# qingpowuwu/emd

Measured on AMD Instinct MI355X. Metric: train iters/s (fwd+bwd) @1066x1600, 2M Gaussians; 1/2/4/8 GPU, higher is better.
Workload: dtype f32

## Files before the change

### emd_amd/csrc/api.hip

```cpp
#include <stdarg.h>
#include <stdio.h>
#include <stdlib.h>
#include <string.h>

#include "common.h"

static thread_local char g_err[512] = "";

void emd_set_error(const char* fmt, ...) {
    va_list ap;
    va_start(ap, fmt);
    vsnprintf(g_err, sizeof(g_err), fmt, ap);
    va_end(ap);
}

#include <mutex>
#include <vector>
namespace {
struct ProfRec { int stage; hipEvent_t a, b; bool b_shared; };
bool g_prof_on = false;
std::mutex g_prof_mu;
std::vector<ProfRec> g_prof_recs;
std::vector<hipEvent_t> g_prof_pool;
hipEvent_t g_prof_open[EMD_PROF_STAGES];
// ... 145 lines not shown
const char* emd_last_error(void) { return g_err; }

int emd_raster_workspace_size(const EmdDims* dims, size_t out[4]) {
    if (!dims || !out) { emd_set_error("workspace_size: null argument"); return EMD_ERR_INVALID; }
    if (dims->num_gaussians < 0 || dims->image_height <= 0 || dims->image_width <= 0 || dims->bin_capacity < 0) {
        emd_set_error("workspace_size: bad dims N=%d H=%d W=%d cap=%lld", dims->num_gaussians, dims->image_height,
                      dims->image_width, (long long)dims->bin_capacity);
        return EMD_ERR_INVALID;
    }
    GeomWs g; BinWs b; ImgWs im;
    const int gx = (dims->image_width + EMD_TILE_X - 1) / EMD_TILE_X, gy = (dims->image_height + EMD_TILE_Y - 1) / EMD_TILE_Y;
    emd_carve_geom(nullptr, dims->num_gaussians, &g);
    emd_carve_bin(nullptr, dims->bin_capacity, gx * gy, &b);
    emd_carve_img(nullptr, dims->image_height, dims->image_width, &im);
    out[0] = g.bytes; out[1] = b.bytes; out[2] = im.bytes;
    if (dims->num_extra < 0 || dims->num_extra > EMD_MAX_EXTRA) { emd_set_error("workspace_size: num_extra %d not in 0..%d", dims->num_extra, EMD_MAX_EXTRA); return EMD_ERR_INVALID; }
    out[3] = (size_t)(dims->num_gaussians > 0 ? dims->num_gaussians : 1) * emd_bwd_stride(dims->num_extra) * sizeof(float);
    return EMD_OK;
}

static int check_common(const EmdSettings& s, int N, int M, const float* means3D, const float* shs,
                        const float* colors, const float* opac, const float* scales, const float* rots,
                        const float* cov, int flags, const EmdMotion& mo) {
    if (N < 0 || s.image_height <= 0 || s.image_width <= 0) { emd_set_error("bad sizes N=%d H=%d W=%d", N, s.image_height, s.image_width); return EMD_ERR_INVALID; }
    if (N > 0 && (!means3D || !opac)) { emd_set_error("means3D / opacities must not be null"); return EMD_ERR_INVALID; }
    if ((shs != nullptr) == (colors != nullptr) && N > 0) { emd_set_error("provide exactly one of shs / colors_precomp"); return EMD_ERR_INVALID; }
    const bool sr = scales && rots;
    if (((scales != nullptr) != (rots != nullptr)) || (sr == (cov != nullptr) && N > 0)) {
        emd_set_error("provide exactly one of (scales, rotations) / cov3D_precomp"); return EMD_ERR_INVALID;
    }
    if (s.sh_degree < 0 || s.sh_degree > 3) { emd_set_error("sh_degree %d not in 0..3", s.sh_degree); return EMD_ERR_INVALID; }
    if (shs && M < (s.sh_degree + 1) * (s.sh_degree + 1)) { emd_set_error("shs holds %d coefficients, degree %d needs %d", M, s.sh_degree, (s.sh_degree + 1) * (s.sh_degree + 1)); return EMD_ERR_INVALID; }
    if (!(flags & EMD_FLAG_SDEV_TANFOV) && (!(s.tanfovx > 0.f) || !(s.tanfovy > 0.f))) { emd_set_error("tanfov must be positive"); return EMD_ERR_INVALID; }
    if (flags & EMD_FLAG_MOTION) {
        if (mo.actor_id && (!mo.actor_pose || mo.num_actors <= 0)) { emd_set_error("motion: actor_id given without actor_pose"); return EMD_ERR_INVALID; }
        if (cov) { emd_set_error("motion: cov3D_precomp cannot be combined with the fused motion transform"); return EMD_ERR_INVALID; }
    }
    if ((flags & EMD_FLAG_RAW_PARAMS) && cov) { emd_set_error("raw params: cov3D_precomp has no raw form"); return EMD_ERR_INVALID; }
    return EMD_OK;
}

int emd_raster_forward(EmdFwdArgs* a, void* hip_stream) {
    if (!a) { emd_set_error("forward: null args"); return EMD_ERR_INVALID; }
    hipStream_t st = (hipStream_t)hip_stream;
    const int N = a->num_gaussians;
    int rc = check_common(a->s, N, a->sh_coeffs, a->means3D, a->shs, a->colors_precomp, a->opacities, a->scales,
                          a->rotations, a->cov3D_precomp, a->flags, a->motion);
    if (rc) return rc;
    if (!a->out_color || !a->out_depth || !a->out_alpha || !a->radii || !a->status || !a->geom_ws || !a->bin_ws || !a->img_ws) {
        emd_set_error("forward: null output / workspace pointer"); return EMD_ERR_INVALID;
    }
    if ((a->flags & EMD_FLAG_NORMAL) && !a->out_normal) { emd_set_error("forward: EMD_FLAG_NORMAL without out_normal"); return EMD_ERR_INVALID; }
    if (a->bin_capacity < 0) { emd_set_error("forward: negative bin_capacity"); return EMD_ERR_INVALID; }
    if ((int64_t)N >= (int64_t)1 << 28) { emd_set_error("forward: %d Gaussians; a list word holds a 28-bit Gaussian id beside the pair's quadrant mask", N); return EMD_ERR_INVALID; }
    if (a->num_extra < 0 || a->num_extra > EMD_MAX_EXTRA) { emd_set_error("forward: num_extra %d not in 0..%d", a->num_extra, EMD_MAX_EXTRA); return EMD_ERR_INVALID; }
    for (int k = 0; k < a->num_extra; k++)
        if (!a->colors_extra[k] || !a->out_extra[k]) { emd_set_error("forward: extra colour set %d: null colours / output", k); return EMD_ERR_INVALID; }
    if ((a->flags & EMD_FLAG_SDEV_TANFOV) && !a->settings_dev) { emd_set_error("forward: EMD_FLAG_SDEV_TANFOV without settings_dev"); return EMD_ERR_INVALID; }
    const int gx = (a->s.image_width + EMD_TILE_X - 1) / EMD_TILE_X, gy = (a->s.image_height + EMD_TILE_Y - 1) / EMD_TILE_Y;
    GeomWs g; BinWs b; ImgWs im;
    emd_carve_geom(a->geom_ws, N, &g);
    emd_carve_bin(a->bin_ws, a->bin_capacity, gx * gy, &b);
    emd_carve_img(a->img_ws, a->s.image_height, a->s.image_width, &im);
    if (g.bytes > a->geom_bytes || b.bytes > a->bin_bytes || im.bytes > a->img_bytes) {
        emd_set_error("forward: workspace too small (geom %zu/%zu bin %zu/%zu img %zu/%zu)", a->geom_bytes, g.bytes,
                      a->bin_bytes, b.bytes, a->img_bytes, im.bytes);
        return EMD_ERR_WORKSPACE;
    }
    const bool dbg = a->s.debug != 0;
#define STAGE_SYNC(name)                                                                                     \
    if (dbg) {                                                                                               \
        hipError_t e_ = hipStreamSynchronize(st);                                                            \
        if (e_ != hipSuccess) { emd_set_error("stage %s failed: %s", name, hipGetErrorString(e_)); return EMD_ERR_HIP; } \
    }
    PreArgs pa;
    pa.s = a->s; pa.N = N; pa.M = a->sh_coeffs; pa.flags = a->flags;
    pa.means3D = a->means3D; pa.shs = a->shs; pa.colors_precomp = a->colors_precomp; pa.opacities = a->opacities;
    pa.scales = a->scales; pa.rotations = a->rotations; pa.cov3D_precomp = a->cov3D_precomp;
    pa.motion = a->motion; pa.radii = a->radii; pa.g = g; pa.status = a->status; pa.sdev = a->settings_dev;
    pa.shs_res0 = a->shs_residual[0]; pa.shs_res1 = a->shs_residual[1];
    if ((pa.shs_res0 || pa.shs_res1) && !a->shs) { emd_set_error("raster_forward: shs_residual needs shs"); return EMD_ERR_INVALID; }
    if (pa.shs_res1 && !pa.shs_res0) { pa.shs_res0 = pa.shs_res1; pa.shs_res1 = nullptr; }
    if (!(a->flags & EMD_FLAG_MOTION)) memset(&pa.motion, 0, sizeof(pa.motion));
    emd_prof_begin(PROF_PREPROCESS, st);
    hipStream_t aux = (hipStream_t)a->aux_stream;
    const bool split = aux != nullptr && aux != st && N > 0 && !dbg;
    hipEvent_t ev_fork = nullptr, ev_join = nullptr;
    auto join = [&]() -> int {
        if (!ev_join) return EMD_OK;
        hipError_t e1 = hipStreamWaitEvent(st, ev_join, 0);
        (void)hipEventDestroy(ev_fork); (void)hipEventDestroy(ev_join);
        ev_fork = ev_join = nullptr;
        if (e1 != hipSuccess) { emd_set_error("forward: joining the auxiliary stream failed: %s", hipGetErrorString(e1)); return EMD_ERR_HIP; }
        return EMD_OK;
    };
    rc = emd_launch_preprocess(pa, split ? 1 : 0, st);
    if (rc) return rc;
    if (split) {
        EMD_HIP_CHECK(hipEventCreateWithFlags(&ev_fork, hipEventDisableTiming));
        EMD_HIP_CHECK(hipEventCreateWithFlags(&ev_join, hipEventDisableTiming));
        EMD_HIP_CHECK(hipEventRecord(ev_fork, st));
        EMD_HIP_CHECK(hipStreamWaitEvent(aux, ev_fork, 0));
        rc = emd_launch_preprocess(pa, 2, aux);
        hipError_t e2 = hipEventRecord(ev_join, aux);
        if (rc || e2 != hipSuccess) { (void)join(); if (!rc) { emd_set_error("forward: hipEventRecord on the auxiliary stream failed"); rc = EMD_ERR_HIP; } return rc; }
    }
    STAGE_SYNC("preprocess");
// ... 306 lines not shown
```

### emd_amd/csrc/footprint.h

```cpp
#pragma once
#include <hip/hip_runtime.h>

struct EllipseCull {
    float mx, my, A, C, kx, ky, nbc, nba, thr;
    bool none, all;
};
__device__ __forceinline__ EllipseCull ellipse_prepare(const float4& r0, const float4& r1) {
    EllipseCull e;
    const float o = r0.w;
    e.mx = r0.x; e.my = r0.y; e.A = r1.x; e.C = r1.z;
    e.none = !(o >= (1.f / 255.f));
    const float ac = r1.x * r1.z, det = ac - r1.y * r1.y;
    e.all = !(det > 0.f) || !(r1.x > 0.f) || !(r1.z > 0.f) || !(det * 3.0e4f > ac);
    e.thr = 2.f * __logf(255.f * o) * 1.01f + 0.05f;
    const float ia = __builtin_amdgcn_rcpf(r1.x), ic = __builtin_amdgcn_rcpf(r1.z);
    e.kx = det * ic; e.ky = det * ia; e.nbc = -r1.y * ic; e.nba = -r1.y * ia;
    return e;
}
__device__ __forceinline__ bool ellipse_hits_rect(const EllipseCull& e, float x0, float x1, float y0, float y1) {
    const float dxa = e.mx - x0, dxb = e.mx - x1, dya = e.my - y0, dyb = e.my - y1;
    const bool inside = dxa >= 0.f && dxb <= 0.f && dya >= 0.f && dyb <= 0.f;
    float ta = e.nbc * dxa, tb = e.nbc * dxb;
    float ea = __builtin_amdgcn_fmed3f(ta, dyb, dya) - ta, eb = __builtin_amdgcn_fmed3f(tb, dyb, dya) - tb;
    const float qa = __builtin_fmaf(e.C * ea, ea, (e.kx * dxa) * dxa), qb = __builtin_fmaf(e.C * eb, eb, (e.kx * dxb) * dxb);
    ta = e.nba * dya; tb = e.nba * dyb;
    ea = __builtin_amdgcn_fmed3f(ta, dxb, dxa) - ta; eb = __builtin_amdgcn_fmed3f(tb, dxb, dxa) - tb;
    const float qc = __builtin_fmaf(e.A * ea, ea, (e.ky * dya) * dya), qd = __builtin_fmaf(e.A * eb, eb, (e.ky * dyb) * dyb);
    const float q = fminf(fminf(qa, qb), fminf(qc, qd));
    return !e.none && (e.all || inside || q <= e.thr);
}
__device__ __forceinline__ uint32_t ellipse_subblock_mask(const float4& r0, const float4& r1, float qx0, float qy0) {
    const EllipseCull e = ellipse_prepare(r0, r1);
    return (ellipse_hits_rect(e, qx0, qx0 + 3.f, qy0, qy0 + 3.f) ? 1u : 0u) | (ellipse_hits_rect(e, qx0 + 4.f, qx0 + 7.f, qy0, qy0 + 3.f) ? 2u : 0u) |
           (ellipse_hits_rect(e, qx0, qx0 + 3.f, qy0 + 4.f, qy0 + 7.f) ? 4u : 0u) |
           (ellipse_hits_rect(e, qx0 + 4.f, qx0 + 7.f, qy0 + 4.f, qy0 + 7.f) ? 8u : 0u);
}
__device__ __forceinline__ uint32_t ellipse_quadrant_mask(const EllipseCull& e, float tx0, float ty0) {
    return (ellipse_hits_rect(e, tx0, tx0 + 7.f, ty0, ty0 + 7.f) ? 1u : 0u) | (ellipse_hits_rect(e, tx0 + 8.f, tx0 + 15.f, ty0, ty0 + 7.f) ? 2u : 0u) |
           (ellipse_hits_rect(e, tx0, tx0 + 7.f, ty0 + 8.f, ty0 + 15.f) ? 4u : 0u) |
           (ellipse_hits_rect(e, tx0 + 8.f, tx0 + 15.f, ty0 + 8.f, ty0 + 15.f) ? 8u : 0u);
}

#define EMD_ID_BITS 28
#define EMD_ID_MASK ((1u << EMD_ID_BITS) - 1u)
```

### emd_amd/csrc/render.hip

```cpp
#include <stdlib.h>

#include <type_traits>

#include "common.h"
#include "device_utils.h"
#include "footprint.h"

namespace {

struct RenderDims {
    int W, H, gx, gy;
    float bg[3];
    const float* bg_dev;
    const float* xcol[EMD_MAX_EXTRA];
    float* xout[EMD_MAX_EXTRA];
    const float* xgrad[EMD_MAX_EXTRA];
};

#define XCD_CHUNK 4
__device__ __forceinline__ uint32_t ordered_quadrant_block(uint32_t b, uint32_t T, const uint32_t* __restrict__ order, uint32_t* quad) {
    const uint32_t xcd = b % 8, k = b / 8, tl = k >> 2;
    *quad = k & 3u;
    const uint32_t pos = tl * 8 + xcd;
    return pos < T ? order[pos] : 0xFFFFFFFFu;
// ... 97 lines not shown
            if (NORMAL) p3 = r[3];
#pragma unroll
            for (int k = 0; k < NX; k++) { const float* c = d.xcol[k] + 3 * (size_t)pgid; px_[k] = make_float4(c[0], c[1], c[2], 0.f); }
        }
    }
    uint32_t* const sv = surv + 4 * (size_t)start + (size_t)quad * n_tile;
    uint32_t total = 0;
    uint32_t scanned = 0;
    while (scanned < n_tile) {
        if (__ballot(!done) == 0ull) break;
        uint32_t head = 0, len0 = 0, len1 = 0, len2 = 0, len3 = 0;
        if (STATS) st_round++;
        while (head <= EMD_WAVE && scanned < n_tile) {
            if (STATS) st_scan++;
            const uint32_t idx = scanned + lane;
            const float4 c0r = p0, c1r = p1, c3r = p3;
            float4 c2r = p2;
            float4 cxr[NX ? NX : 1];
#pragma unroll
            for (int k = 0; k < NX; k++) cxr[k] = px_[k];
            const uint32_t cgid = pgid;
            const bool keep = pkeep;
            {
                const uint32_t w = w_nxt;
                w_nxt = (idx + 2 * EMD_WAVE < n_tile) ? point_list[start + idx + 2 * EMD_WAVE] : 0u;
                pkeep = (w & qbit) != 0u;
                pgid = w & EMD_ID_MASK;
                if (pkeep) {
                    const float4* r = rec + (size_t)pgid * EMD_REC_F4;
                    p0 = r[0]; p1 = r[1]; p2 = r[2];
                    if (NORMAL) p3 = r[3];
#pragma unroll
                    for (int k = 0; k < NX; k++) { const float* c = d.xcol[k] + 3 * (size_t)pgid; px_[k] = make_float4(c[0], c[1], c[2], 0.f); }
                }
            }
            const unsigned long long bal = __ballot(keep);
            const uint32_t slot = head + (uint32_t)__popcll(bal & lt);
            if (keep) {
                c2r.w = __uint_as_float(cgid);
                s0[slot] = c0r; s1[slot] = c1r; s2[slot] = c2r;
                if (NORMAL) s3[slot] = c3r;
#pragma unroll
                for (int k = 0; k < NX; k++) sx[k][slot] = cxr[k];
            }
            head += (uint32_t)__popcll(bal);
            scanned += EMD_WAVE;
        }
        __syncthreads();
        for (uint32_t base = 0; base < head; base += EMD_WAVE) {
            if (STATS) st_cull++;
            const uint32_t slot = base + lane;
            uint32_t m4 = 0u, gid = 0u;
            if (slot < head) { gid = __float_as_uint(reinterpret_cast<const float*>(&s2[slot])[3]); m4 = ellipse_subblock_mask(s0[slot], s1[slot], qx0, qy0); }
            const unsigned long long b0 = __ballot(m4 & 1u), b1 = __ballot(m4 & 2u), b2 = __ballot(m4 & 4u), b3 = __ballot(m4 & 8u);
            const unsigned long long ba = b0 | b1 | b2 | b3;
            if (m4) {
                const uint32_t num = total + (uint32_t)__popcll(ba & lt);
                sv[num] = gid;
                reinterpret_cast<float*>(&s2[slot])[3] = __uint_as_float(num + 1);
            }
            total += (uint32_t)__popcll(ba);
            if (m4 & 1u) s_list[0][len0 + (uint32_t)__popcll(b0 & lt)] = (uint8_t)slot;
            if (m4 & 2u) s_list[1][len1 + (uint32_t)__popcll(b1 & lt)] = (uint8_t)slot;
            if (m4 & 4u) s_list[2][len2 + (uint32_t)__popcll(b2 & lt)] = (uint8_t)slot;
            if (m4 & 8u) s_list[3][len3 + (uint32_t)__popcll(b3 & lt)] = (uint8_t)slot;
            len0 += (uint32_t)__popcll(b0); len1 += (uint32_t)__popcll(b1); len2 += (uint32_t)__popcll(b2); len3 += (uint32_t)__popcll(b3);
        }
        __syncthreads();
        const uint32_t nmax = max(max(len0, len1), max(len2, len3));
        if (STATS) { st_drain += nmax; st_useful += len0 + len1 + len2 + len3; }
        if (nmax) {
            const uint32_t n = row == 0 ? len0 : row == 1 ? len1 : row == 2 ? len2 : len3;
            const uint8_t* list = s_list[row];
            uint32_t j = n ? list[0] : 0u;
            float4 g0 = s0[j], g1 = s1[j];
#pragma unroll 2
            for (uint32_t i = 0; i < nmax; i++) {
                const bool active = i < n;
                const uint32_t jn = (i + 1 < n) ? list[i + 1] : j;
                const float4 g0n = s0[jn], g1n = s1[jn];
                const float dx = g0.x - pfx, dy = g0.y - pfy;
                const float power = gauss_power(g1.x, g1.y, g1.z, dx, dy);
                const float alpha = fminf(0.99f, g0.w * pinned_exp(power));
                const bool hit = active && !done && power <= 0.f && alpha >= (1.f / 255.f);
                const float test_T = T * (1.f - alpha);
                const bool stop = hit && test_T < 0.0001f;
                const bool take = hit && !stop;
                const float w = take ? alpha * T : 0.f;
                const float4 g2 = s2[j];
                C0 = __builtin_fmaf(g2.x, w, C0); C1 = __builtin_fmaf(g2.y, w, C1); C2 = __builtin_fmaf(g2.z, w, C2);
                Dz = __builtin_fmaf(g0.z, w, Dz);
                if (NORMAL) {
                    const float4 g3 = s3[j];
                    N0 = __builtin_fmaf(g3.x, w, N0); N1 = __builtin_fmaf(g3.y, w, N1); N2 = __builtin_fmaf(g3.z, w, N2);
                }
#pragma unroll
                for (int k = 0; k < NX; k++) {
                    const float4 gx = sx[k][j];
                    X[k][0] = __builtin_fmaf(gx.x, w, X[k][0]); X[k][1] = __builtin_fmaf(gx.y, w, X[k][1]); X[k][2] = __builtin_fmaf(gx.z, w, X[k][2]);
                }
                T = take ? test_T : T;
                last = take ? __float_as_uint(g2.w) : last;
                done = done || stop;
                j = jn; g0 = g0n; g1 = g1n;
            }
        }
        __syncthreads();
    }
    if (inside) {
        const size_t HW = (size_t)d.H * d.W, pix = (size_t)py * d.W + px;
        out_color[pix] = __builtin_fmaf(T, bg0, C0);
        out_color[HW + pix] = __builtin_fmaf(T, bg1, C1);
        out_color[2 * HW + pix] = __builtin_fmaf(T, bg2, C2);
        out_depth[pix] = Dz;
        if (NORMAL) { out_normal[pix] = N0; out_normal[HW + pix] = N1; out_normal[2 * HW + pix] = N2; }
#pragma unroll
        for (int k = 0; k < NX; k++) {
            d.xout[k][pix] = __builtin_fmaf(T, bg0, X[k][0]);
            d.xout[k][HW + pix] = __builtin_fmaf(T, bg1, X[k][1]);
            d.xout[k][2 * HW + pix] = __builtin_fmaf(T, bg2, X[k][2]);
        }
        out_alpha[pix] = 1.f - T;
        final_T[pix] = T;
        n_contrib[pix] = last;
    }
    uint32_t need = inside ? last : 0u;
    for (int off = 32; off; off >>= 1) need = max(need, (uint32_t)__shfl_xor((int)need, off));
    if (lane == 0) quad_need[4 * tile + quad] = need;
    if (STATS && lane == 0) {
        atomicAdd(loop_stats, st_scan); atomicAdd(loop_stats + 1, st_cull); atomicAdd(loop_stats + 2, st_drain); atomicAdd(loop_stats + 3, st_useful);
        atomicAdd(loop_stats + 4, st_round); atomicAdd(loop_stats + 5, 1ull);
    }
}


#define BQ_QUEUE 128

template <bool NORMAL, bool ABS, int NX, bool STATS = false>
__global__ void __launch_bounds__(EMD_WAVE) __attribute__((amdgpu_waves_per_eu(NX == 0 ? 4 : NX == 1 ? 3 : 2))) k_render_backward_q(RenderDims d, const uint32_t* __restrict__ tile_order, const uint32_t* __restrict__ ranges,
                                                                const uint32_t* __restrict__ surv,
                                                                const uint32_t* __restrict__ quad_need,
                                                                const float4* __restrict__ rec,
                                                                const float* __restrict__ final_T,
                                                                const uint32_t* __restrict__ n_contrib,
                                                                const float* __restrict__ out_color,
                                                                const float* __restrict__ out_depth,
                                                                const float* __restrict__ out_normal,
                                                                const float* __restrict__ dL_dcolor,
                                                                const float* __restrict__ dL_ddepth,
                                                                const float* __restrict__ dL_dalpha,
                                                                const float* __restrict__ dL_dnormal,
                                                                float* __restrict__ grad_rec,
                                                                float* __restrict__ zero_buf, int zero_n,
                                                                unsigned long long* __restrict__ pair_stats) {
    if (blockIdx.x == 0)
        for (int i = threadIdx.x; i < zero_n; i += EMD_WAVE) zero_buf[i] = 0.f;
    constexpr int STRIDE = EMD_BWD_PAYLOAD + 4 * NX;
    constexpr int PITCH = emd_bwd_stride(NX);
    constexpr int PB = NORMAL ? 6 : 4;
    __shared__ float4 s_stage4[EMD_WAVE * STRIDE / 4];
    __shared__ uint32_t q_id[EMD_WAVE];
    float* const s_stage = reinterpret_cast<float*>(s_stage4);
    __shared__ float4 s_pix[EMD_WAVE / 2][PB + 2 * NX];
    __shared__ uint32_t s_myn[EMD_WAVE];
    uint32_t quad;
    const uint32_t tile = ordered_quadrant_block(blockIdx.x, (uint32_t)(d.gx * d.gy), tile_order, &quad);
    if (tile >= (uint32_t)(d.gx * d.gy)) return;
    const uint32_t lane = threadIdx.x;
    const float tile_x0 = (float)((tile % (uint32_t)d.gx) * EMD_TILE_X), tile_y0 = (float)((tile / (uint32_t)d.gx) * EMD_TILE_Y);
    const float qx0 = tile_x0 + (float)((quad & 1) * 8), qy0 = tile_y0 + (float)((quad >> 1) * 8);
    const int px = (int)qx0 + (int)(lane & 7), py = (int)qy0 + (int)(lane >> 3);
    const bool inside = px < d.W && py < d.H;
    const uint32_t start = ranges[2 * tile], n_tile = ranges[2 * tile + 1] - start;
    const uint32_t wave_n = min(quad_need[4 * tile + quad], n_tile);
    if (wave_n == 0) return;
    const uint32_t* const sv = surv + 4 * (size_t)start + (size_t)quad * n_tile;
    const size_t HW = (size_t)d.H * d.W, pix = (size_t)py * d.W + px;
    const uint32_t my_n = inside ? n_contrib[pix] : 0u;
    s_myn[lane] = my_n;
    float dC0 = 0.f, dC1 = 0.f, dC2 = 0.f, dD = 0.f, dN0 = 0.f, dN1 = 0.f, dN2 = 0.f, Q = 0.f, Tf = 1.f;
    float dX[NX ? NX : 1][3];
#pragma unroll
    for (int k = 0; k < (NX ? NX : 1); k++) dX[k][0] = dX[k][1] = dX[k][2] = 0.f;
    if (inside) {
        float dA = 0.f;
#ifndef K7_ABL_NO_PROLOGUE
        Tf = final_T[pix];
        if (dL_dcolor) { dC0 = dL_dcolor[pix]; dC1 = dL_dcolor[HW + pix]; dC2 = dL_dcolor[2 * HW + pix]; }
        if (dL_ddepth) dD = dL_ddepth[pix];
        if (dL_dalpha) dA = dL_dalpha[pix];
#else
        Tf = 0.37f; dC0 = 1e-6f; dC1 = -2e-6f; dC2 = 3e-6f;
#endif
        if (NORMAL && dL_dnormal) { dN0 = dL_dnormal[pix]; dN1 = dL_dnormal[HW + pix]; dN2 = dL_dnormal[2 * HW + pix]; }
        const float bg0 = d.bg_dev ? d.bg_dev[0] : d.bg[0], bg1 = d.bg_dev ? d.bg_dev[1] : d.bg[1], bg2 = d.bg_dev ? d.bg_dev[2] : d.bg[2];
        float bgdot = bg0 * dC0 + bg1 * dC1 + bg2 * dC2;
#pragma unroll
        for (int k = 0; k < NX; k++) {
            if (!d.xgrad[k]) continue;
            dX[k][0] = d.xgrad[k][pix]; dX[k][1] = d.xgrad[k][HW + pix]; dX[k][2] = d.xgrad[k][2 * HW + pix];
            bgdot += bg0 * dX[k][0] + bg1 * dX[k][1] + bg2 * dX[k][2];
        }
        Q = Tf * (dA - bgdot);
    }
    {
        float* sp = reinterpret_cast<float*>(&s_pix[lane >> 1][0]) + (lane & 1);
        sp[0] = dC0; sp[2] = dC1; sp[4] = dC2; sp[6] = dD;
        sp[8] = Tf; sp[10] = 0.f;
        sp[12] = Q; sp[14] = 0.f;
        if (NORMAL) { sp[16] = dN0; sp[18] = dN1; sp[20] = dN2; sp[22] = 0.f; }
#pragma unroll
        for (int k = 0; k < NX; k++) { float* sx_ = sp + 4 * (PB + 2 * k); sx_[0] = dX[k][0]; sx_[2] = dX[k][1]; sx_[4] = dX[k][2]; sx_[6] = 0.f; }
    }
    __syncthreads();
    const float4 zero4 = make_float4(0.f, 0.f, 0.f, 0.f);
    unsigned long long st_eval = 0ull, st_hit = 0ull, st_rows = 0ull, st_atoms = 0ull;

    auto process_batch = [&](auto half_c, uint32_t nb, const float4 g0, const float4 g1, const float4 g2, const float4 g3, const float4* gxc, uint32_t pos,
                             uint32_t gid) {
        constexpr bool HALF = decltype(half_c)::value;
        const uint32_t el = HALF ? (lane & 31u) : lane, hp = HALF ? (lane >> 5) : 0u;
        const bool valid = el < nb;
        v2f xr_2[NX ? NX : 1], xg_2[NX ? NX : 1], xb_2[NX ? NX : 1];
#pragma unroll
        for (int k = 0; k < (NX ? NX : 1); k++) xr_2[k] = xg_2[k] = xb_2[k] = splat2(0.f);
        const uint32_t last_pos = readlane_u32(pos, (int)nb - 1);
        const v2f z2 = splat2(0.f);
        v2f m0_2 = z2, gx_2 = z2, gy_2 = z2, m2xx_2 = z2, m2xy_2 = z2, m2yy_2 = z2, dz_2 = z2, r_2 = z2, g_2 = z2, b_2 = z2;
        float a_ax = 0.f, a_ay = 0.f;
        for (int pp0 = 0; pp0 < (HALF ? EMD_WAVE / 4 : EMD_WAVE / 2); pp0++) {
            const int pp = HALF ? pp0 + (int)(hp * (EMD_WAVE / 4)) : pp0;
            uint32_t n_a, n_b;
            if (HALF) {
                n_a = s_myn[2 * pp]; n_b = s_myn[2 * pp + 1];
                if (__ballot(max(n_a, n_b) > last_pos) == 0ull) continue;
            } else {
                n_a = readlane_u32(my_n, 2 * pp); n_b = readlane_u32(my_n, 2 * pp + 1);
                if (max(n_a, n_b) <= last_pos) continue;
            }
            const float4 c01 = s_pix[pp][0], c2d = s_pix[pp][1], ts = s_pix[pp][2], qq = s_pix[pp][3];
            const float pxs = qx0 + (float)((2 * pp) & 7), pys = qy0 + (float)(pp >> 2);
            const float dy = g0.y - pys;
            const v2f dx = (v2f){g0.x - pxs, g0.x - (pxs + 1.f)};
            const v2f power = gauss_power2(g1.x, g1.y, g1.z, dx, dy);
            const v2f G = pinned_exp2(power);
            const v2f aw = splat2(g0.w) * G;
            const v2f alpha = (v2f){fminf(0.99f, aw.x), fminf(0.99f, aw.y)};
            const bool hit_a = valid && pos < n_a && power.x <= 0.f && alpha.x >= (1.f / 255.f);
            const bool hit_b = valid && pos < n_b && power.y <= 0.f && alpha.y >= (1.f / 255.f);
            if (STATS) { st_eval += (HALF ? 4ull : 2ull) * nb; st_hit += (unsigned long long)(__popcll(__ballot(hit_a)) + __popcll(__ballot(hit_b))); }
            if (__ballot(hit_a || hit_b) == 0ull) continue;
            const v2f a = (v2f){hit_a ? alpha.x : 0.f, hit_b ? alpha.y : 0.f};
            const v2f om = splat2(1.f) - a;
            const v2f inv = (v2f){__builtin_amdgcn_rcpf(om.x), __builtin_amdgcn_rcpf(om.y)};
            float t_a = inv.x, t_b = inv.y;
            if (HALF) half_scan_mul2_f32_asm(t_a, t_b); else wave_scan_mul2_f32_asm(t_a, t_b);
            const v2f cT = (v2f){ts.x, ts.y}, cR = (v2f){ts.z, ts.w};
            const v2f Tk = cT * (v2f){t_a, t_b};
            const v2f w = a * Tk;
            v2f g = splat2(g2.x) * (v2f){c01.x, c01.y} + splat2(g2.y) * (v2f){c01.z, c01.w} + splat2(g2.z) * (v2f){c2d.x, c2d.y} +
                    splat2(g0.z) * (v2f){c2d.z, c2d.w};
            if (NORMAL) {
                const float4 n01 = s_pix[pp][4], n2 = s_pix[pp][5];
                g += splat2(g3.x) * (v2f){n01.x, n01.y} + splat2(g3.y) * (v2f){n01.z, n01.w} + splat2(g3.z) * (v2f){n2.x, n2.y};
            }
            float4 x01[NX ? NX : 1], x2_[NX ? NX : 1];
#pragma unroll
            for (int k = 0; k < NX; k++) {
                x01[k] = s_pix[pp][PB + 2 * k]; x2_[k] = s_pix[pp][PB + 2 * k + 1];
                g += splat2(gxc[k].x) * (v2f){x01[k].x, x01[k].y} + splat2(gxc[k].y) * (v2f){x01[k].z, x01[k].w} + splat2(gxc[k].z) * (v2f){x2_[k].x, x2_[k].y};
            }
            const v2f gw = g * w;
            float s_a = gw.x, s_b = gw.y;
            if (HALF) half_scan_add2_f32_asm(s_a, s_b); else wave_scan_add2_f32_asm(s_a, s_b);
            float ex_a = wave_shift_up1_f32(s_a, 0.f), ex_b = wave_shift_up1_f32(s_b, 0.f);
            if (HALF && lane == 32u) { ex_a = 0.f; ex_b = 0.f; }
            const v2f Rk = cR + (v2f){ex_a, ex_b};
            v2f dL_da = g * Tk + inv * ((v2f){qq.x, qq.y} - Rk);
            dL_da = (v2f){hit_a ? dL_da.x : 0.f, hit_b ? dL_da.y : 0.f};
            const v2f u = G * (splat2(g0.w) * dL_da);
            const v2f ux = u * dx, uy = u * splat2(dy);
            const v2f tx = __builtin_elementwise_fma(splat2(g1.x), dx, splat2(g1.y * dy));
            const v2f ty = __builtin_elementwise_fma(splat2(g1.y), dx, splat2(g1.z * dy));
            const v2f ax = u * tx, ay = u * ty;
            m0_2 += u; gx_2 += ax; gy_2 += ay;
            m2xx_2 += ux * dx; m2xy_2 += ux * splat2(dy); m2yy_2 += uy * splat2(dy);
            if (ABS) { a_ax += fabsf(ax.x) + fabsf(ax.y); a_ay += fabsf(ay.x) + fabsf(ay.y); }
            dz_2 += w * (v2f){c2d.z, c2d.w};
            r_2 += w * (v2f){c01.x, c01.y}; g_2 += w * (v2f){c01.z, c01.w}; b_2 += w * (v2f){c2d.x, c2d.y};
#pragma unroll
            for (int k = 0; k < NX; k++) {
                xr_2[k] += w * (v2f){x01[k].x, x01[k].y}; xg_2[k] += w * (v2f){x01[k].z, x01[k].w}; xb_2[k] += w * (v2f){x2_[k].x, x2_[k].y};
            }
            if ((lane & (HALF ? 31u : 63u)) == (HALF ? 31u : 63u)) s_pix[pp][2] = make_float4(cT.x * t_a, cT.y * t_b, cR.x + s_a, cR.y + s_b);
        }
        if (HALF) {
            auto fold = [](v2f& x) { x.x += __shfl_xor(x.x, 32); x.y += __shfl_xor(x.y, 32); };
            fold(m0_2); fold(gx_2); fold(gy_2); fold(m2xx_2); fold(m2xy_2); fold(m2yy_2); fold(dz_2); fold(r_2); fold(g_2); fold(b_2);
            if (ABS) { a_ax += __shfl_xor(a_ax, 32); a_ay += __shfl_xor(a_ay, 32); }
#pragma unroll
            for (int k = 0; k < NX; k++) { fold(xr_2[k]); fold(xg_2[k]); fold(xb_2[k]); }
        }
        const float m0 = m0_2.x + m0_2.y, gx = gx_2.x + gx_2.y, gy = gy_2.x + gy_2.y, m2xx = m2xx_2.x + m2xx_2.y,
                    m2xy = m2xy_2.x + m2xy_2.y, m2yy = m2yy_2.x + m2yy_2.y, a_dz = dz_2.x + dz_2.y, a_r = r_2.x + r_2.y,
                    a_g = g_2.x + g_2.y, a_b = b_2.x + b_2.y;
        q_id[lane] = gid;
        float4* row = reinterpret_cast<float4*>(s_stage + lane * STRIDE);
        row[0] = make_float4(-gx, -gy, a_dz, m0 * __builtin_amdgcn_rcpf(g0.w));
        row[1] = make_float4(-0.5f * m2xx, -m2xy, -0.5f * m2yy, a_r);
        row[2] = make_float4(a_g, a_b, ABS ? a_ax : 0.f, ABS ? a_ay : 0.f);
#pragma unroll
        for (int k = 0; k < NX; k++) row[3 + k] = make_float4(xr_2[k].x + xr_2[k].y, xg_2[k].x + xg_2[k].y, xb_2[k].x + xb_2[k].y, 0.f);
        __syncthreads();
        if (STATS) {
            bool nz = false;
            if (lane < nb)
                for (int v = 0; v < STRIDE; v++) nz = nz || s_stage[lane * STRIDE + v] != 0.f;
            st_rows += (unsigned long long)__popcll(__ballot(nz));
        }
        static_assert(EMD_WAVE % PITCH == 0, "a row is a whole number of 16-lane groups");
        {
            const uint32_t v = lane % PITCH;
            if (v < (uint32_t)STRIDE)
                for (uint32_t e = lane / PITCH; e < nb; e += EMD_WAVE / PITCH) {
                    const float val = s_stage[e * STRIDE + v];
                    if (STATS) st_atoms += (unsigned long long)__popcll(__ballot(val != 0.f));
#ifndef K7_ABL_NO_FLUSH
                    if (val != 0.f) atomicAdd(grad_rec + (size_t)q_id[e] * PITCH + v, val);
#else
                    if (val == 12345.678f) grad_rec[0] = val;
#endif
                }
        }
        __syncthreads();
    };

    const int steps = (int)((wave_n + EMD_WAVE - 1) / EMD_WAVE);
    auto step_lo = [&](int st_) -> int { return (steps - 1 - st_) * EMD_WAVE; };
    auto step_idx = [&](int st_) -> int { return st_ < steps ? min((int)wave_n, step_lo(st_) + EMD_WAVE) - 1 - (int)lane : -1; };
    auto in_step = [&](int st_, int i) -> bool { return st_ < steps && i >= step_lo(st_); };
    auto load_id = [&](int st_) -> uint32_t { const int i = step_idx(st_); return in_step(st_, i) ? sv[i] : 0u; };
    float4 a0 = zero4, a1 = zero4, a2 = zero4, a3 = zero4, b0 = zero4, b1 = zero4, b2 = zero4, b3 = zero4;
    float4 ax_[NX ? NX : 1], bx_[NX ? NX : 1];
#pragma unroll
    for (int k = 0; k < (NX ? NX : 1); k++) ax_[k] = bx_[k] = zero4;
    auto load_extra = [&](uint32_t id, float4* o) {
#pragma unroll
        for (int k = 0; k < NX; k++) { const float* c = d.xcol[k] + 3 * (size_t)id; o[k] = make_float4(c[0], c[1], c[2], 0.f); }
    };
    uint32_t idA = load_id(0), idB = load_id(1), idC = load_id(2);
    if (in_step(0, step_idx(0))) {
        const float4* r = rec + (size_t)idA * EMD_REC_F4;
        a0 = r[0]; a1 = r[1]; a2 = r[2];
        if (NORMAL) a3 = r[3];
        load_extra(idA, ax_);
    }
    if (in_step(1, step_idx(1))) {
        const float4* r = rec + (size_t)idB * EMD_REC_F4;
        b0 = r[0]; b1 = r[1]; b2 = r[2];
        if (NORMAL) b3 = r[3];
        load_extra(idB, bx_);
    }
    for (int st_ = 0; st_ < steps; st_++) {
        const int idx = step_idx(st_);
        const float4 c0r = a0, c1r = a1, c2r = a2, c3r = a3;
        float4 cxr[NX ? NX : 1];
#pragma unroll
        for (int k = 0; k < NX; k++) { cxr[k] = ax_[k]; ax_[k] = bx_[k]; }
        const uint32_t cid = idA;
        a0 = b0; a1 = b1; a2 = b2; a3 = b3; idA = idB;
        idB = idC;
        b0 = b1 = b2 = b3 = zero4;
#pragma unroll
        for (int k = 0; k < NX; k++) bx_[k] = zero4;
        if (in_step(st_ + 2, step_idx(st_ + 2))) {
            const float4* r = rec + (size_t)idB * EMD_REC_F4;
            b0 = r[0]; b1 = r[1]; b2 = r[2];
            if (NORMAL) b3 = r[3];
            load_extra(idB, bx_);
        }
        idC = load_id(st_ + 3);
        const uint32_t nb = (uint32_t)(min((int)wave_n, step_lo(st_) + EMD_WAVE) - step_lo(st_));
        if (nb <= EMD_WAVE / 2) {
            const int src = (int)(lane & 31u);
            auto dup4 = [&](float4 v) { return make_float4(__shfl(v.x, src), __shfl(v.y, src), __shfl(v.z, src), __shfl(v.w, src)); };
            const float4 h0 = dup4(c0r), h1 = dup4(c1r), h2 = dup4(c2r), h3 = NORMAL ? dup4(c3r) : c3r;
            float4 hx[NX ? NX : 1];
#pragma unroll
            for (int k = 0; k < NX; k++) hx[k] = dup4(cxr[k]);
            process_batch(std::true_type{}, nb, h0, h1, h2, h3, hx, (uint32_t)__shfl(max(idx, 0), src), (uint32_t)__shfl((int)cid, src));
        } else {
            process_batch(std::false_type{}, nb, c0r, c1r, c2r, c3r, cxr, (uint32_t)max(idx, 0), cid);
        }
    }
    if (STATS && lane == 0) { atomicAdd(pair_stats, st_eval); atomicAdd(pair_stats + 1, st_hit); atomicAdd(pair_stats + 2, st_rows); atomicAdd(pair_stats + 3, st_atoms); }
}

RenderDims make_dims(const EmdSettings& s, const float* sdev, const EmdExtra* x) {
    RenderDims d;
    d.bg_dev = sdev;
    d.W = s.image_width; d.H = s.image_height;
    d.gx = (d.W + EMD_TILE_X - 1) / EMD_TILE_X; d.gy = (d.H + EMD_TILE_Y - 1) / EMD_TILE_Y;
    d.bg[0] = s.bg[0]; d.bg[1] = s.bg[1]; d.bg[2] = s.bg[2];
    for (int k = 0; k < EMD_MAX_EXTRA; k++) {
        const bool on = x && k < x->num;
        d.xcol[k] = on ? x->colors[k] : nullptr;
        d.xout[k] = on ? x->out[k] : nullptr;
        d.xgrad[k] = on ? x->dL_dout[k] : nullptr;
    }
    return d;
}

}

int emd_launch_render_forward(const EmdSettings& s, const float* sdev, int flags, const GeomWs& g, const BinWs& b, const ImgWs& im,
                              float* out_color, float* out_depth, float* out_normal, float* out_alpha, const EmdExtra* x,
                              unsigned long long* loop_stats, hipStream_t st) {
    const RenderDims d = make_dims(s, sdev, x);
    const int T = d.gx * d.gy;
    if (T <= 0) return EMD_OK;
    const uint32_t* pl = b.vals[b.sorted_buf];
    const int nx = x ? x->num : 0;
#define LAUNCH_FWD(N_, X_)                                                                                                          \
    hipLaunchKernelGGL((k_render_forward_q<N_, X_>), dim3(4 * padded_tile_grid(T)), dim3(EMD_WAVE), 0, st, d, b.tile_order, b.ranges, pl, g.rec, \
                       out_color, out_depth, out_normal, out_alpha, im.final_T, im.n_contrib, b.surv, b.quad_need, nullptr)
    const bool nrm = (flags & EMD_FLAG_NORMAL) != 0;
    if (nx == 0 && loop_stats) {
        if (nrm) hipLaunchKernelGGL((k_render_forward_q<true, 0, true>), dim3(4 * padded_tile_grid(T)), dim3(EMD_WAVE), 0, st, d, b.tile_order, b.ranges, pl, g.rec,
                                    out_color, out_depth, out_normal, out_alpha, im.final_T, im.n_contrib, b.surv, b.quad_need, loop_stats);
        else hipLaunchKernelGGL((k_render_forward_q<false, 0, true>), dim3(4 * padded_tile_grid(T)), dim3(EMD_WAVE), 0, st, d, b.tile_order, b.ranges, pl, g.rec,
                                out_color, out_depth, out_normal, out_alpha, im.final_T, im.n_contrib, b.surv, b.quad_need, loop_stats);
    }
    else if (nx == 0) { if (nrm) LAUNCH_FWD(true, 0); else LAUNCH_FWD(false, 0); }
    else if (nx == 1) { if (nrm) LAUNCH_FWD(true, 1); else LAUNCH_FWD(false, 1); }
    else { if (nrm) LAUNCH_FWD(true, 2); else LAUNCH_FWD(false, 2); }
#undef LAUNCH_FWD
    EMD_LAUNCH_CHECK();
    return EMD_OK;
}

int emd_launch_render_backward(const EmdSettings& s, const float* sdev, int flags, const GeomWs& g, const BinWs& b, const ImgWs& im,
                               const float* out_color, const float* out_depth, const float* out_normal,
                               const float* dL_dcolor, const float* dL_ddepth, const float* dL_dalpha,
                               const float* dL_dnormal, const EmdExtra* x, float* grad_rec, float* zero_buf, int zero_n,
                               unsigned long long* pair_stats, hipStream_t st) {
    const RenderDims d = make_dims(s, sdev, x);
// ... 27 lines not shown
```

Before: 909.4.

## Split backward survivor lists by quadrant half and compact per-half ring queues

```diff
diff --git a/emd_amd/csrc/api.hip b/emd_amd/csrc/api.hip
--- a/emd_amd/csrc/api.hip
+++ b/emd_amd/csrc/api.hip
@@ -221,7 +221,7 @@
     }
     if ((a->flags & EMD_FLAG_NORMAL) && !a->out_normal) { emd_set_error("forward: EMD_FLAG_NORMAL without out_normal"); return EMD_ERR_INVALID; }
     if (a->bin_capacity < 0) { emd_set_error("forward: negative bin_capacity"); return EMD_ERR_INVALID; }
-    if ((int64_t)N >= (int64_t)1 << 28) { emd_set_error("forward: %d Gaussians; a list word holds a 28-bit Gaussian id beside the pair's quadrant mask", N); return EMD_ERR_INVALID; }
+    if ((int64_t)N >= (int64_t)1 << 28) { emd_set_error("forward: %d Gaussians; a list word holds a 28-bit Gaussian id beside the pair's quadrant mask, a survivor word beside its two half bits", N); return EMD_ERR_INVALID; }
     if (a->num_extra < 0 || a->num_extra > EMD_MAX_EXTRA) { emd_set_error("forward: num_extra %d not in 0..%d", a->num_extra, EMD_MAX_EXTRA); return EMD_ERR_INVALID; }
     for (int k = 0; k < a->num_extra; k++)
         if (!a->colors_extra[k] || !a->out_extra[k]) { emd_set_error("forward: extra colour set %d: null colours / output", k); return EMD_ERR_INVALID; }
diff --git a/emd_amd/csrc/footprint.h b/emd_amd/csrc/footprint.h
--- a/emd_amd/csrc/footprint.h
+++ b/emd_amd/csrc/footprint.h
@@ -43,3 +43,5 @@
 
 #define EMD_ID_BITS 28
 #define EMD_ID_MASK ((1u << EMD_ID_BITS) - 1u)
+#define EMD_SURV_TOP (1u << 30)
+#define EMD_SURV_BOTTOM (1u << 31)
diff --git a/emd_amd/csrc/render.hip b/emd_amd/csrc/render.hip
--- a/emd_amd/csrc/render.hip
+++ b/emd_amd/csrc/render.hip
@@ -173,18 +173,20 @@
             const uint32_t slot = base + lane;
             uint32_t m4 = 0u, gid = 0u;
             if (slot < head) { gid = __float_as_uint(reinterpret_cast<const float*>(&s2[slot])[3]); m4 = ellipse_subblock_mask(s0[slot], s1[slot], qx0, qy0); }
-            const unsigned long long b0 = __ballot(m4 & 1u), b1 = __ballot(m4 & 2u), b2 = __ballot(m4 & 4u), b3 = __ballot(m4 & 8u);
+            auto below = [](unsigned long long bal, uint32_t base) { return __builtin_amdgcn_mbcnt_hi((uint32_t)(bal >> 32), __builtin_amdgcn_mbcnt_lo((uint32_t)bal, base)); };
+            const bool h0 = m4 & 1u, h1 = m4 & 2u, h2 = m4 & 4u, h3 = m4 & 8u;
+            const unsigned long long b0 = __ballot(h0), b1 = __ballot(h1), b2 = __ballot(h2), b3 = __ballot(h3);
             const unsigned long long ba = b0 | b1 | b2 | b3;
             if (m4) {
-                const uint32_t num = total + (uint32_t)__popcll(ba & lt);
-                sv[num] = gid;
+                const uint32_t num = below(ba, total);
+                sv[num] = gid | ((h0 || h1) ? EMD_SURV_TOP : 0u) | ((h2 || h3) ? EMD_SURV_BOTTOM : 0u);
                 reinterpret_cast<float*>(&s2[slot])[3] = __uint_as_float(num + 1);
             }
             total += (uint32_t)__popcll(ba);
-            if (m4 & 1u) s_list[0][len0 + (uint32_t)__popcll(b0 & lt)] = (uint8_t)slot;
-            if (m4 & 2u) s_list[1][len1 + (uint32_t)__popcll(b1 & lt)] = (uint8_t)slot;
-            if (m4 & 4u) s_list[2][len2 + (uint32_t)__popcll(b2 & lt)] = (uint8_t)slot;
-            if (m4 & 8u) s_list[3][len3 + (uint32_t)__popcll(b3 & lt)] = (uint8_t)slot;
+            if (h0) s_list[0][below(b0, len0)] = (uint8_t)slot;
+            if (h1) s_list[1][below(b1, len1)] = (uint8_t)slot;
+            if (h2) s_list[2][below(b2, len2)] = (uint8_t)slot;
+            if (h3) s_list[3][below(b3, len3)] = (uint8_t)slot;
             len0 += (uint32_t)__popcll(b0); len1 += (uint32_t)__popcll(b1); len2 += (uint32_t)__popcll(b2); len3 += (uint32_t)__popcll(b3);
         }
         __syncthreads();
@@ -255,7 +257,7 @@
 }
 
 
-#define BQ_QUEUE 128
+#define BQ_RING 64u
 
 template <bool NORMAL, bool ABS, int NX, bool STATS = false>
 __global__ void __launch_bounds__(EMD_WAVE) __attribute__((amdgpu_waves_per_eu(NX == 0 ? 4 : NX == 1 ? 3 : 2))) k_render_backward_q(RenderDims d, const uint32_t* __restrict__ tile_order, const uint32_t* __restrict__ ranges,
@@ -281,13 +283,14 @@
     constexpr int PB = NORMAL ? 6 : 4;
     __shared__ float4 s_stage4[EMD_WAVE * STRIDE / 4];
     __shared__ uint32_t q_id[EMD_WAVE];
+    __shared__ uint32_t r_id[2][BQ_RING], r_pos[2][BQ_RING];
     float* const s_stage = reinterpret_cast<float*>(s_stage4);
     __shared__ float4 s_pix[EMD_WAVE / 2][PB + 2 * NX];
     __shared__ uint32_t s_myn[EMD_WAVE];
     uint32_t quad;
     const uint32_t tile = ordered_quadrant_block(blockIdx.x, (uint32_t)(d.gx * d.gy), tile_order, &quad);
     if (tile >= (uint32_t)(d.gx * d.gy)) return;
-    const uint32_t lane = threadIdx.x;
+    const uint32_t lane = threadIdx.x, hp = lane >> 5, el = lane & 31u;
     const float tile_x0 = (float)((tile % (uint32_t)d.gx) * EMD_TILE_X), tile_y0 = (float)((tile / (uint32_t)d.gx) * EMD_TILE_Y);
     const float qx0 = tile_x0 + (float)((quad & 1) * 8), qy0 = tile_y0 + (float)((quad >> 1) * 8);
     const int px = (int)qx0 + (int)(lane & 7), py = (int)qy0 + (int)(lane >> 3);
@@ -337,28 +340,21 @@
     const float4 zero4 = make_float4(0.f, 0.f, 0.f, 0.f);
     unsigned long long st_eval = 0ull, st_hit = 0ull, st_rows = 0ull, st_atoms = 0ull;
 
-    auto process_batch = [&](auto half_c, uint32_t nb, const float4 g0, const float4 g1, const float4 g2, const float4 g3, const float4* gxc, uint32_t pos,
-                             uint32_t gid) {
-        constexpr bool HALF = decltype(half_c)::value;
-        const uint32_t el = HALF ? (lane & 31u) : lane, hp = HALF ? (lane >> 5) : 0u;
+    auto process_batch = [&](uint32_t nb, const float4 g0, const float4 g1, const float4 g2, const float4 g3, const float4* gxc, uint32_t pos, uint32_t gid) {
         const bool valid = el < nb;
         v2f xr_2[NX ? NX : 1], xg_2[NX ? NX : 1], xb_2[NX ? NX : 1];
 #pragma unroll
         for (int k = 0; k < (NX ? NX : 1); k++) xr_2[k] = xg_2[k] = xb_2[k] = splat2(0.f);
-        const uint32_t last_pos = readlane_u32(pos, (int)nb - 1);
+        const uint32_t nb_t = readlane_u32(nb, 0), nb_b = readlane_u32(nb, 32);
+        const uint32_t lp_t = nb_t ? readlane_u32(pos, (int)nb_t - 1) : 0xFFFFFFFFu, lp_b = nb_b ? readlane_u32(pos, 32 + (int)nb_b - 1) : 0xFFFFFFFFu;
+        const uint32_t last_pos = hp ? lp_b : lp_t;
         const v2f z2 = splat2(0.f);
         v2f m0_2 = z2, gx_2 = z2, gy_2 = z2, m2xx_2 = z2, m2xy_2 = z2, m2yy_2 = z2, dz_2 = z2, r_2 = z2, g_2 = z2, b_2 = z2;
         float a_ax = 0.f, a_ay = 0.f;
-        for (int pp0 = 0; pp0 < (HALF ? EMD_WAVE / 4 : EMD_WAVE / 2); pp0++) {
-            const int pp = HALF ? pp0 + (int)(hp * (EMD_WAVE / 4)) : pp0;
-            uint32_t n_a, n_b;
-            if (HALF) {
-                n_a = s_myn[2 * pp]; n_b = s_myn[2 * pp + 1];
-                if (__ballot(max(n_a, n_b) > last_pos) == 0ull) continue;
-            } else {
-                n_a = readlane_u32(my_n, 2 * pp); n_b = readlane_u32(my_n, 2 * pp + 1);
-                if (max(n_a, n_b) <= last_pos) continue;
-            }
+        for (int pp0 = 0; pp0 < EMD_WAVE / 4; pp0++) {
+            const int pp = pp0 + (int)(hp * (EMD_WAVE / 4));
+            const uint32_t n_a = s_myn[2 * pp], n_b = s_myn[2 * pp + 1];
+            if (__ballot(max(n_a, n_b) > last_pos) == 0ull) continue;
             const float4 c01 = s_pix[pp][0], c2d = s_pix[pp][1], ts = s_pix[pp][2], qq = s_pix[pp][3];
             const float pxs = qx0 + (float)((2 * pp) & 7), pys = qy0 + (float)(pp >> 2);
             const float dy = g0.y - pys;
@@ -369,13 +365,13 @@
             const v2f alpha = (v2f){fminf(0.99f, aw.x), fminf(0.99f, aw.y)};
             const bool hit_a = valid && pos < n_a && power.x <= 0.f && alpha.x >= (1.f / 255.f);
             const bool hit_b = valid && pos < n_b && power.y <= 0.f && alpha.y >= (1.f / 255.f);
-            if (STATS) { st_eval += (HALF ? 4ull : 2ull) * nb; st_hit += (unsigned long long)(__popcll(__ballot(hit_a)) + __popcll(__ballot(hit_b))); }
+            if (STATS) { st_eval += 2ull * (nb_t + nb_b); st_hit += (unsigned long long)(__popcll(__ballot(hit_a)) + __popcll(__ballot(hit_b))); }
             if (__ballot(hit_a || hit_b) == 0ull) continue;
             const v2f a = (v2f){hit_a ? alpha.x : 0.f, hit_b ? alpha.y : 0.f};
             const v2f om = splat2(1.f) - a;
             const v2f inv = (v2f){__builtin_amdgcn_rcpf(om.x), __builtin_amdgcn_rcpf(om.y)};
             float t_a = inv.x, t_b = inv.y;
-            if (HALF) half_scan_mul2_f32_asm(t_a, t_b); else wave_scan_mul2_f32_asm(t_a, t_b);
+            half_scan_mul2_f32_asm(t_a, t_b);
             const v2f cT = (v2f){ts.x, ts.y}, cR = (v2f){ts.z, ts.w};
             const v2f Tk = cT * (v2f){t_a, t_b};
             const v2f w = a * Tk;
@@ -393,9 +389,9 @@
             }
             const v2f gw = g * w;
             float s_a = gw.x, s_b = gw.y;
-            if (HALF) half_scan_add2_f32_asm(s_a, s_b); else wave_scan_add2_f32_asm(s_a, s_b);
+            half_scan_add2_f32_asm(s_a, s_b);
             float ex_a = wave_shift_up1_f32(s_a, 0.f), ex_b = wave_shift_up1_f32(s_b, 0.f);
-            if (HALF && lane == 32u) { ex_a = 0.f; ex_b = 0.f; }
+            if (lane == 32u) { ex_a = 0.f; ex_b = 0.f; }
             const v2f Rk = cR + (v2f){ex_a, ex_b};
             v2f dL_da = g * Tk + inv * ((v2f){qq.x, qq.y} - Rk);
             dL_da = (v2f){hit_a ? dL_da.x : 0.f, hit_b ? dL_da.y : 0.f};
@@ -413,19 +409,12 @@
             for (int k = 0; k < NX; k++) {
                 xr_2[k] += w * (v2f){x01[k].x, x01[k].y}; xg_2[k] += w * (v2f){x01[k].z, x01[k].w}; xb_2[k] += w * (v2f){x2_[k].x, x2_[k].y};
             }
-            if ((lane & (HALF ? 31u : 63u)) == (HALF ? 31u : 63u)) s_pix[pp][2] = make_float4(cT.x * t_a, cT.y * t_b, cR.x + s_a, cR.y + s_b);
-        }
-        if (HALF) {
-            auto fold = [](v2f& x) { x.x += __shfl_xor(x.x, 32); x.y += __shfl_xor(x.y, 32); };
-            fold(m0_2); fold(gx_2); fold(gy_2); fold(m2xx_2); fold(m2xy_2); fold(m2yy_2); fold(dz_2); fold(r_2); fold(g_2); fold(b_2);
-            if (ABS) { a_ax += __shfl_xor(a_ax, 32); a_ay += __shfl_xor(a_ay, 32); }
-#pragma unroll
-            for (int k = 0; k < NX; k++) { fold(xr_2[k]); fold(xg_2[k]); fold(xb_2[k]); }
+            if (el == 31u) s_pix[pp][2] = make_float4(cT.x * t_a, cT.y * t_b, cR.x + s_a, cR.y + s_b);
         }
         const float m0 = m0_2.x + m0_2.y, gx = gx_2.x + gx_2.y, gy = gy_2.x + gy_2.y, m2xx = m2xx_2.x + m2xx_2.y,
                     m2xy = m2xy_2.x + m2xy_2.y, m2yy = m2yy_2.x + m2yy_2.y, a_dz = dz_2.x + dz_2.y, a_r = r_2.x + r_2.y,
                     a_g = g_2.x + g_2.y, a_b = b_2.x + b_2.y;
-        q_id[lane] = gid;
+        q_id[lane] = valid ? gid : 0xFFFFFFFFu;
         float4* row = reinterpret_cast<float4*>(s_stage + lane * STRIDE);
         row[0] = make_float4(-gx, -gy, a_dz, m0 * __builtin_amdgcn_rcpf(g0.w));
         row[1] = make_float4(-0.5f * m2xx, -m2xy, -0.5f * m2yy, a_r);
@@ -435,19 +424,20 @@
         __syncthreads();
         if (STATS) {
             bool nz = false;
-            if (lane < nb)
+            if (valid)
                 for (int v = 0; v < STRIDE; v++) nz = nz || s_stage[lane * STRIDE + v] != 0.f;
             st_rows += (unsigned long long)__popcll(__ballot(nz));
         }
         static_assert(EMD_WAVE % PITCH == 0, "a row is a whole number of 16-lane groups");
         {
-            const uint32_t v = lane % PITCH;
+            const uint32_t v = lane % PITCH, row_end = nb_b ? EMD_WAVE / 2 + nb_b : nb_t;
             if (v < (uint32_t)STRIDE)
-                for (uint32_t e = lane / PITCH; e < nb; e += EMD_WAVE / PITCH) {
-                    const float val = s_stage[e * STRIDE + v];
+                for (uint32_t e = lane / PITCH; e < row_end; e += EMD_WAVE / PITCH) {
+                    const uint32_t id = q_id[e];
+                    const float val = id != 0xFFFFFFFFu ? s_stage[e * STRIDE + v] : 0.f;
                     if (STATS) st_atoms += (unsigned long long)__popcll(__ballot(val != 0.f));
 #ifndef K7_ABL_NO_FLUSH
-                    if (val != 0.f) atomicAdd(grad_rec + (size_t)q_id[e] * PITCH + v, val);
+                    if (val != 0.f) atomicAdd(grad_rec + (size_t)id * PITCH + v, val);
 #else
                     if (val == 12345.678f) grad_rec[0] = val;
 #endif
@@ -456,63 +446,55 @@
         __syncthreads();
     };
 
-    const int steps = (int)((wave_n + EMD_WAVE - 1) / EMD_WAVE);
-    auto step_lo = [&](int st_) -> int { return (steps - 1 - st_) * EMD_WAVE; };
-    auto step_idx = [&](int st_) -> int { return st_ < steps ? min((int)wave_n, step_lo(st_) + EMD_WAVE) - 1 - (int)lane : -1; };
-    auto in_step = [&](int st_, int i) -> bool { return st_ < steps && i >= step_lo(st_); };
-    auto load_id = [&](int st_) -> uint32_t { const int i = step_idx(st_); return in_step(st_, i) ? sv[i] : 0u; };
-    float4 a0 = zero4, a1 = zero4, a2 = zero4, a3 = zero4, b0 = zero4, b1 = zero4, b2 = zero4, b3 = zero4;
-    float4 ax_[NX ? NX : 1], bx_[NX ? NX : 1];
-#pragma unroll
-    for (int k = 0; k < (NX ? NX : 1); k++) ax_[k] = bx_[k] = zero4;
-    auto load_extra = [&](uint32_t id, float4* o) {
-#pragma unroll
-        for (int k = 0; k < NX; k++) { const float* c = d.xcol[k] + 3 * (size_t)id; o[k] = make_float4(c[0], c[1], c[2], 0.f); }
+    uint32_t rd = wave_n, cnt = 0u, head = 0u;
+    const uint32_t hbit = hp ? EMD_SURV_BOTTOM : EMD_SURV_TOP, lt32 = (1u << el) - 1u;
+    auto word_at = [&](uint32_t rd_) -> uint32_t { return sv[rd_ > el ? rd_ - 1u - el : 0u]; };
+    uint32_t w_pf = word_at(rd);
+    auto fill = [&]() {
+        for (;;) {
+            const bool want = cnt < EMD_WAVE / 2 && rd > 0u;
+            if (__ballot(want) == 0ull) break;
+            const bool keep = want && rd > el && (w_pf & hbit) != 0u;
+            const unsigned long long bal = __ballot(keep);
+            const uint32_t hb = hp ? (uint32_t)(bal >> 32) : (uint32_t)bal;
+            if (keep) {
+                const uint32_t slot = (head + cnt + (uint32_t)__popc(hb & lt32)) & (BQ_RING - 1u);
+                r_id[hp][slot] = w_pf & EMD_ID_MASK; r_pos[hp][slot] = rd - 1u - el;
+            }
+            cnt += (uint32_t)__popc(hb);
+            rd = want ? (rd > EMD_WAVE / 2 ? rd - EMD_WAVE / 2 : 0u) : rd;
+            w_pf = word_at(rd);
+        }
+        __syncthreads();
     };
-    uint32_t idA = load_id(0), idB = load_id(1), idC = load_id(2);
-    if (in_step(0, step_idx(0))) {
-        const float4* r = rec + (size_t)idA * EMD_REC_F4;
-        a0 = r[0]; a1 = r[1]; a2 = r[2];
-        if (NORMAL) a3 = r[3];
-        load_extra(idA, ax_);
-    }
-    if (in_step(1, step_idx(1))) {
-        const float4* r = rec + (size_t)idB * EMD_REC_F4;
-        b0 = r[0]; b1 = r[1]; b2 = r[2];
-        if (NORMAL) b3 = r[3];
-        load_extra(idB, bx_);
-    }
-    for (int st_ = 0; st_ < steps; st_++) {
-        const int idx = step_idx(st_);
-        const float4 c0r = a0, c1r = a1, c2r = a2, c3r = a3;
-        float4 cxr[NX ? NX : 1];
-#pragma unroll
-        for (int k = 0; k < NX; k++) { cxr[k] = ax_[k]; ax_[k] = bx_[k]; }
-        const uint32_t cid = idA;
-        a0 = b0; a1 = b1; a2 = b2; a3 = b3; idA = idB;
-        idB = idC;
-        b0 = b1 = b2 = b3 = zero4;
-#pragma unroll
-        for (int k = 0; k < NX; k++) bx_[k] = zero4;
-        if (in_step(st_ + 2, step_idx(st_ + 2))) {
-            const float4* r = rec + (size_t)idB * EMD_REC_F4;
-            b0 = r[0]; b1 = r[1]; b2 = r[2];
-            if (NORMAL) b3 = r[3];
-            load_extra(idB, bx_);
-        }
-        idC = load_id(st_ + 3);
-        const uint32_t nb = (uint32_t)(min((int)wave_n, step_lo(st_) + EMD_WAVE) - step_lo(st_));
-        if (nb <= EMD_WAVE / 2) {
-            const int src = (int)(lane & 31u);
-            auto dup4 = [&](float4 v) { return make_float4(__shfl(v.x, src), __shfl(v.y, src), __shfl(v.z, src), __shfl(v.w, src)); };
-            const float4 h0 = dup4(c0r), h1 = dup4(c1r), h2 = dup4(c2r), h3 = NORMAL ? dup4(c3r) : c3r;
-            float4 hx[NX ? NX : 1];
-#pragma unroll
-            for (int k = 0; k < NX; k++) hx[k] = dup4(cxr[k]);
-            process_batch(std::true_type{}, nb, h0, h1, h2, h3, hx, (uint32_t)__shfl(max(idx, 0), src), (uint32_t)__shfl((int)cid, src));
-        } else {
-            process_batch(std::false_type{}, nb, c0r, c1r, c2r, c3r, cxr, (uint32_t)max(idx, 0), cid);
-        }
+    float4 a0, a1, a2, a3 = zero4, ax_[NX ? NX : 1];
+#pragma unroll
+    for (int k = 0; k < (NX ? NX : 1); k++) ax_[k] = zero4;
+    uint32_t nbA, idA, posA;
+    auto take = [&](uint32_t& nb, uint32_t& id, uint32_t& pos, float4& r0, float4& r1, float4& r2, float4& r3, float4* rx) {
+        nb = min(cnt, (uint32_t)(EMD_WAVE / 2));
+        const uint32_t slot = (head + el) & (BQ_RING - 1u);
+        id = el < nb ? r_id[hp][slot] : 0u; pos = el < nb ? r_pos[hp][slot] : 0u;
+        head = (head + nb) & (BQ_RING - 1u); cnt -= nb;
+        const float4* r = rec + (size_t)id * EMD_REC_F4;
+        r0 = r[0]; r1 = r[1]; r2 = r[2];
+        if (NORMAL) r3 = r[3];
+#pragma unroll
+        for (int k = 0; k < NX; k++) { const float* c = d.xcol[k] + 3 * (size_t)id; rx[k] = make_float4(c[0], c[1], c[2], 0.f); }
+    };
+    fill();
+    take(nbA, idA, posA, a0, a1, a2, a3, ax_);
+    while (__ballot(nbA != 0u) != 0ull) {
+        float4 b0, b1, b2, b3 = zero4, bx_[NX ? NX : 1];
+#pragma unroll
+        for (int k = 0; k < (NX ? NX : 1); k++) bx_[k] = zero4;
+        uint32_t nbB, idB, posB;
+        fill();
+        take(nbB, idB, posB, b0, b1, b2, b3, bx_);
+        process_batch(nbA, a0, a1, a2, a3, ax_, posA, idA);
+        a0 = b0; a1 = b1; a2 = b2; a3 = b3; nbA = nbB; idA = idB; posA = posB;
+#pragma unroll
+        for (int k = 0; k < NX; k++) ax_[k] = bx_[k];
     }
     if (STATS && lane == 0) { atomicAdd(pair_stats, st_eval); atomicAdd(pair_stats + 1, st_hit); atomicAdd(pair_stats + 2, st_rows); atomicAdd(pair_stats + 3, st_atoms); }
 }
```

New measurement: 840.6. -7.6%, worse.
